# fabianschenk/REVO

Hardware: AMD Instinct MI355X
Metric: tracked frames/sec at 640x480, 4-level pyramid; ATE vs reference (higher is better)
Workload: dtype f32

## Files before the change

revo_amd/csrc/revo_dev.h:

```cpp
#pragma once
#include <hip/hip_runtime.h>
#include <stdint.h>
#include "../../include/revo_hip.h"

#define REVO_L REVO_MAX_LEVELS

struct LevelGeom {
  int w, h;
  int npix;
  float fx, fy, cx, cy;
  int patch;
  int hist_w, hist_h;
  int nchunk;
  int chunk_rows;
  int wpr;
  int nms_block_base;
  int has_orig;
  int pix_base;
  int edt_rows;
  int edt_block_base;
  int strip_base;
  int cc_base;
  int band_rows, nbands, band_base;
};

struct PyrGeom {
  int frame0;
  int n_levels;
  int total_nms_blocks, total_pix, total_edt_blocks, total_strips, total_cc;
  int total_bands, any_banded;
  int hyst_force;
  int hyst_heavy_runs;
  int total_tiles;
  int pts_staged;
  float depth_min, depth_max;
  int canny_low, canny_high;
  int use_edge_hist;
  float n_percentage;
  double fill_thr[REVO_L];
  LevelGeom lv[REVO_L];
};

struct FramePlanes {
  uint8_t* gray[REVO_L];
  float* depth[REVO_L];
  uint2* cs[REVO_L];
  uint8_t* edges[REVO_L];
  uint8_t* edges_orig[REVO_L];
  int* scratch[REVO_L];
  float4* pts[REVO_L];
  float4* pts_trk[REVO_L];
  float* dt[REVO_L];
  float4* table[REVO_L];
  uint8_t* hist[REVO_L];
  int* chunk[REVO_L];
  unsigned* cmask[REVO_L];
  uint8_t* vb[REVO_L];
  int* npts;
  int* hist_nz;
  int* strip_tot;
  uint32_t* ebits[REVO_L];
  int* need_full;
  int* hyst_heavy;
  int* tile_base;
  float* stage[REVO_L];
  unsigned short* epre[REVO_L];
  int* stage_base;
};

struct PairDesc {
  const float4* pts[REVO_L];
  const int* npts;
  const float* dt[REVO_L];
  float R[9];
  float T[3];
};

struct TrackParams {
  int pyr_min_lvl, pyr_max_lvl;
  int lvl_begin, lvl_end;
  int check_init;
  int eval_only;
  int kspec[REVO_L];
  int redundant_n;
  float lambda_success_fac, lambda_fail_fac;
  float lambda_initial[REVO_L], step_size_min[REVO_L], convergence_eps[REVO_L];
  int max_its[REVO_L];
  float edge_distance[REVO_L];
  float huber_edge;
  int use_edge_filter;
  struct { float fx, fy, cx, cy; int w, h; } cam[REVO_L];
  int exact_sums;
};

struct EvalOut {
  float A[36];
  float b[6];
  float error;
  float mean_err;
  float sum_w, sum_u;
  int good, bad;
};

#define REVO_MAX_WIDTH 2048
#define NMS_ROWS 6
#define EDT_ROW_PX 1280
#ifndef REVO_HYST_LDS_MAX
#define REVO_HYST_LDS_MAX 158720
#endif
#ifndef TRACK_THREADS
#define TRACK_THREADS 512
#endif
#ifndef TRACK_MAX_CLUSTER
#define TRACK_MAX_CLUSTER 32
#endif
#define TRACK_KMAX 4
#define TRACK_NVAL 48
#define TRACK_NVAL_X 132
#define TRACK_MAIL_NVAL TRACK_NVAL_X

void launch_gray_depth(const PyrGeom& g, const FramePlanes& p, const uint8_t* d_bgr, const float* d_depth_f32,
                       const uint16_t* d_depth_u16, float u16_alpha, int B, hipStream_t s);
void launch_pyrdown(const PyrGeom& g, const FramePlanes& p, int lvl, int B, hipStream_t s, int parts = 3, bool stage_edges = false);
void launch_edge_prefix(const PyrGeom& g, const FramePlanes& p, int B, hipStream_t s);
void launch_canny_nms(const PyrGeom& g, const FramePlanes& p, int B, hipStream_t s);
void launch_hyst(const PyrGeom& g, const FramePlanes& p, int B, hipStream_t s);
void launch_fill(const PyrGeom& g, const FramePlanes& p, int B, hipStream_t s);
void launch_compact(const PyrGeom& g, const FramePlanes& p, int B, hipStream_t s);
void launch_tile_points(const PyrGeom& g, const FramePlanes& p, int B, hipStream_t s, int which = 3);
void launch_pyrdown_bgr(const uint8_t* src, int w, int h, uint8_t* dst, hipStream_t s);
void launch_colored_pcl(const PyrGeom& g, const FramePlanes& p, int frame, int lvl, int dense, const uint8_t* bgr_lvl,
                        int* chunk, unsigned* cmask, int* total, int cap, float* out8, hipStream_t s);
void launch_keyframe(const PyrGeom& g, const FramePlanes& p, int f0, int fstride, int count, hipStream_t s, int which = 3);
int launch_track(const PairDesc* d_descs, const TrackParams& prm, revo_pair_result* d_out, EvalOut* d_eval,
                 int n_pairs, unsigned long long* d_mail, unsigned* epoch_io, int cluster, unsigned* d_resident, hipStream_t s);
void launch_track_gate(unsigned* d_resident, unsigned want, hipStream_t s);
int launch_track_one(const PairDesc& desc, const TrackParams& prm, revo_pair_result* out, EvalOut* eval_out,
                     unsigned long long* d_mail, unsigned* epoch_io, int cluster, unsigned* seq_ptr, unsigned seq_val,
                     unsigned* d_resident, hipStream_t s);
void launch_solve6(const float* d_Ab , int n, float* d_x , hipStream_t s);
int track_blocks_per_cu();
void launch_grad_table(const PyrGeom& g, const FramePlanes& p, int f0, int fstride, int count, hipStream_t s);
struct VoteArgs { float RT[3][12]; const float4* pts[3]; const int* n[3]; };
void launch_vote(const PyrGeom& g, const FramePlanes& curr, int curr_frame, int lvl, int n_clouds, const VoteArgs& va,
                 int* d_marks , int* d_hist8 , unsigned* d_done ,
                 int* h_out8 , unsigned seq_val, int use_orig_edges,
                 hipStream_t s);
void launch_copy_cloud(float4* dst, const float4* src, int* dst_n, const int* src_n, hipStream_t s);
struct VoteDesc {
  float RT[3][12]; const float4* pts[3]; const int* n[3]; int n_clouds;
  const uint8_t* edges; const float* depth;
  int* marks; int* hist8; unsigned* done;
  int* host_out;
};
struct CloudCopyDesc { float4* dst; const float4* src; int* dst_n; const int* src_n; };
struct CopySeg { const void* src; void* dst; size_t bytes; };
void launch_vote_multi(const PyrGeom& g, int lvl, int n, const VoteDesc* d_descs, unsigned seq_val, hipStream_t s);
void launch_copy_cloud_multi(int n, const CloudCopyDesc* d_descs, hipStream_t s);
void launch_copy_segments(int n, const CopySeg* d_segs, hipStream_t s);
```

revo_amd/csrc/revo_pyramid.hip:

```cpp
#include "revo_dev.h"
#include <type_traits>

namespace {

#ifdef REVO_BUILD_PRIO
#define BUILD_PRIO() __builtin_amdgcn_s_setprio(REVO_BUILD_PRIO)
#else
#define BUILD_PRIO()
#endif

__device__ __forceinline__ int level_of(const PyrGeom& g, int v, int LevelGeom::*base) {
  int l = 0;
#pragma unroll
  for (int k = 1; k < REVO_L; ++k)
    if (k < g.n_levels && v >= g.lv[k].*base) l = k;
  return l;
}
__device__ __forceinline__ int clampi(int v, int lo, int hi) { return v < lo ? lo : (v > hi ? hi : v); }
__device__ __forceinline__ int reflect101(int i, int n) {
  if (i < 0) i = -i;
  if (i >= n) i = 2 * n - 2 - i;
  return i;
}

// ... 74 lines not shown
    if (GRAY && r < 2 * nrows + 3) {
      const uint32_t* row = srcw + (size_t)reflect101(2 * oy - 2 + r, sh) * swords;
      uint32_t w0 = row[max(w1i - 1, 0)];
      const uint32_t w1 = row[w1i], w2 = row[w1i + 1];
      uint32_t w3 = row[min(w1i + 2, swords - 1)];
      if (gx == 0) w0 = (((w1 >> 16) & 0xffu) << 16) | (((w1 >> 8) & 0xffu) << 24);
      if (gx == gw - 1) w3 = (w2 >> 16) & 0xffu;
      const int b[11] = {(int)((w0 >> 16) & 0xffu), (int)(w0 >> 24),
                         (int)(w1 & 0xffu), (int)((w1 >> 8) & 0xffu), (int)((w1 >> 16) & 0xffu), (int)(w1 >> 24),
                         (int)(w2 & 0xffu), (int)((w2 >> 8) & 0xffu), (int)((w2 >> 16) & 0xffu), (int)(w2 >> 24),
                         (int)(w3 & 0xffu)};
#pragma unroll
      for (int j = 0; j < 4; ++j) hs[r][j] = b[2 * j] + b[2 * j + 4] + 4 * (b[2 * j + 1] + b[2 * j + 3]) + 6 * b[2 * j + 2];
    } else {
#pragma unroll
      for (int j = 0; j < 4; ++j) hs[r][j] = 0;
    }
  }
#pragma unroll
  for (int q = 0; q < 2; ++q) {
    if (q >= nrows) break;
    if (GRAY) {
      uint32_t packed = 0;
#pragma unroll
      for (int j = 0; j < 4; ++j) {
        const int v = hs[2 * q][j] + hs[2 * q + 4][j] + 4 * (hs[2 * q + 1][j] + hs[2 * q + 3][j]) + 6 * hs[2 * q + 2][j];
        packed |= (uint32_t)((v + 128) >> 8) << (8 * j);
      }
      reinterpret_cast<uint32_t*>(dst + (size_t)(oy + q) * dw)[gx] = packed;
    }
    if (!DEPTH) continue;
    const float* d0 = dsrc + (size_t)(2 * (oy + q)) * sw + 8 * gx;
    const float4 a0 = *reinterpret_cast<const float4*>(d0), a1 = *reinterpret_cast<const float4*>(d0 + 4);
    const float4 c0 = *reinterpret_cast<const float4*>(d0 + sw), c1 = *reinterpret_cast<const float4*>(d0 + sw + 4);
    const float top[8] = {a0.x, a0.y, a0.z, a0.w, a1.x, a1.y, a1.z, a1.w};
    const float bot[8] = {c0.x, c0.y, c0.z, c0.w, c1.x, c1.y, c1.z, c1.w};
    unsigned vt = 0, vbm = 0;
#pragma unroll
    for (int k = 0; k < 8; ++k) {
      vt |= (isfinite(top[k]) && top[k] > dmin && top[k] < dmax) ? 1u << k : 0u;
      vbm |= (isfinite(bot[k]) && bot[k] > dmin && bot[k] < dmax) ? 1u << k : 0u;
    }
    vsrc[(size_t)(2 * (oy + q)) * (sw >> 3) + gx] = (uint8_t)vt;
    vsrc[(size_t)(2 * (oy + q) + 1) * (sw >> 3) + gx] = (uint8_t)vbm;
    if (STAGE) {
      const int wc = (8 * gx) >> 5, sh8 = (8 * gx) & 31;
#pragma unroll
      for (int rr = 0; rr < 2; ++rr) {
        const int y = 2 * (oy + q) + rr;
        const uint32_t E = es.cs[((size_t)f * sh + y) * es.wpr + wc].y;
        uint32_t eb = (E >> sh8) & 0xffu;
        if (eb) {
          const int tile = (y >> 5) * es.wpr + wc;
          int pos = es.base[(size_t)f * es.tiles_total + tile] + (int)es.epre[((size_t)f * sh + y) * es.wpr + wc] +
                    __popc(E & ((1u << sh8) - 1u));
          float* o = es.out + (size_t)f * sw * sh;
          const float* row = rr ? bot : top;
#pragma unroll
          for (int k = 0; k < 8; ++k)
            if ((eb >> k) & 1u) o[pos++] = row[k];
        }
      }
    }
    float o[4];
#pragma unroll
    for (int j = 0; j < 4; ++j) {
      float out = 0.0f, cnt = 0.0f;
      if (top[2 * j] > 0.0f) { out += top[2 * j]; cnt += 1.0f; }
      if (top[2 * j + 1] > 0.0f) { out += top[2 * j + 1]; cnt += 1.0f; }
      if (bot[2 * j] > 0.0f) { out += bot[2 * j]; cnt += 1.0f; }
      if (bot[2 * j + 1] > 0.0f) { out += bot[2 * j + 1]; cnt += 1.0f; }
      if (cnt > 0.0f) out = __fdiv_rn(out, cnt);
      o[j] = out;
    }
    *reinterpret_cast<float4*>(ddst + (size_t)(oy + q) * dw + 4 * gx) = make_float4(o[0], o[1], o[2], o[3]);
  }
}

typedef short s2v __attribute__((ext_vector_type(2)));
__device__ __forceinline__ s2v as_s2(uint32_t v) { return __builtin_bit_cast(s2v, v); }
__device__ __forceinline__ uint32_t as_u32(s2v v) { return __builtin_bit_cast(uint32_t, v); }
#define PAIR(hi, lo, sel) as_s2(__builtin_amdgcn_perm((hi), (lo), (sel)))

__device__ __forceinline__ void nms_px(int k, int aL, int aM, int aR, int bL, int m, int bR, int cL, int cM, int cR, uint32_t dxy,
                                       int low, int high, uint32_t& cb, uint32_t& sb) {
  const int TG22 = 13573;
  const s2v v = as_s2(dxy);
  const s2v z = {0, 0};
  const uint32_t ab = as_u32(__builtin_elementwise_max(v, z - v));
  const int ax = (int)(ab & 0xffffu);
  const int ay15 = (int)((ab >> 1) & 0x7fff8000u);
  const int t22 = ax * TG22;
  const bool horiz = ay15 < t22;
  const bool vert = ay15 > t22 + (ax << 16);
  const bool neg = (int)(dxy ^ (dxy << 16)) < 0;
  const int diag_a = neg ? aR : aL;
  const int diag_b = neg ? cL : cR;
  const int a = horiz ? bL : (vert ? aM : diag_a);
  const int b = horiz ? bR : (vert ? cM : diag_b);
  const bool ge = horiz || vert;
  const bool is_max = (m > a) & (ge ? (m >= b) : (m > b));
  const bool c = (m > low) & is_max;
  cb |= c ? (1u << k) : 0u;
  sb |= (c & (m > high)) ? (1u << k) : 0u;
}
#define NMS_R 6

struct HRow4 { s2v d[3], s[3]; };
__device__ __forceinline__ HRow4 hrow4(uint32_t prev, uint32_t m0, uint32_t next) {
  const s2v E0 = PAIR(0u, prev, 0x0c030c02u), E1 = PAIR(0u, m0, 0x0c010c00u), E2 = PAIR(0u, m0, 0x0c030c02u), E3 = PAIR(0u, next, 0x0c010c00u);
  const s2v O0 = PAIR(m0, prev, 0x0c040c03u), O1 = PAIR(0u, m0, 0x0c020c01u), O2 = PAIR(next, m0, 0x0c040c03u);
  HRow4 r;
  r.d[0] = E1 - E0; r.d[1] = E2 - E1; r.d[2] = E3 - E2;
  r.s[0] = (E0 + E1) + (O0 + O0); r.s[1] = (E1 + E2) + (O1 + O1); r.s[2] = (E2 + E3) + (O2 + O2);
  return r;
}
struct MRow4 { int v0, v1, v2, v3, v4, v5; };
struct DRow4 { uint32_t v0, v1, v2, v3; };
__device__ __forceinline__ void mag_row4(const HRow4& a, const HRow4& b, const HRow4& c, uint32_t cm_left, uint32_t cm_right, bool valid,
                                         MRow4& m, DRow4& dxy) {
  uint32_t lo[3], hi[3];
#pragma unroll
  for (int k = 0; k < 3; ++k) {
    const s2v dx = (a.d[k] + c.d[k]) + (b.d[k] + b.d[k]);
    const s2v dy = c.s[k] - a.s[k];
    lo[k] = __builtin_amdgcn_perm(as_u32(dy), as_u32(dx), 0x05040100u);
    hi[k] = __builtin_amdgcn_perm(as_u32(dy), as_u32(dx), 0x07060302u);
  }
  const uint32_t rv = valid ? ~0u : 0u;
#define MAG2(x) __builtin_amdgcn_sdot2(as_s2(x), as_s2(x), 0, false)
  m.v0 = MAG2(lo[0]) & (int)(cm_left & rv);
  m.v1 = MAG2(hi[0]) & (int)rv;
  m.v2 = MAG2(lo[1]) & (int)rv;
  m.v3 = MAG2(hi[1]) & (int)rv;
  m.v4 = MAG2(lo[2]) & (int)rv;
  m.v5 = MAG2(hi[2]) & (int)(cm_right & rv);
#undef MAG2
  dxy.v0 = hi[0]; dxy.v1 = lo[1]; dxy.v2 = hi[1]; dxy.v3 = lo[2];
}
__device__ __forceinline__ void nms_row4(const MRow4& A, const MRow4& B, const MRow4& C, const DRow4& d, int low, int high,
                                         uint32_t* cand, uint32_t* strong) {
  uint32_t cb = 0, sb = 0;
  nms_px(0, A.v0, A.v1, A.v2, B.v0, B.v1, B.v2, C.v0, C.v1, C.v2, d.v0, low, high, cb, sb);
  nms_px(1, A.v1, A.v2, A.v3, B.v1, B.v2, B.v3, C.v1, C.v2, C.v3, d.v1, low, high, cb, sb);
  nms_px(2, A.v2, A.v3, A.v4, B.v2, B.v3, B.v4, C.v2, C.v3, C.v4, d.v2, low, high, cb, sb);
  nms_px(3, A.v3, A.v4, A.v5, B.v3, B.v4, B.v5, C.v3, C.v4, C.v5, d.v3, low, high, cb, sb);
  *cand = cb;
  *strong = sb;
}
__global__ void __launch_bounds__(256) k_canny_nms4(PyrGeom g, FramePlanes pl) {
  BUILD_PRIO();
  const int f = g.frame0 + blockIdx.z;
  if (blockIdx.x == 0 && threadIdx.x < REVO_L) {
    pl.need_full[f * REVO_L + threadIdx.x] = 0;
    pl.hist_nz[f * REVO_L + threadIdx.x] = 0;
  }
  const int l = level_of(g, blockIdx.x, &LevelGeom::nms_block_base);
  const LevelGeom& lv = g.lv[l];
  const int w = lv.w, h = lv.h;
  const int rt = 8 * lv.wpr;
  const int t = (blockIdx.x - lv.nms_block_base) * 256 + threadIdx.x;
  const int yb = t / rt, xg = t - yb * rt;
  const int y0 = yb * NMS_R;
  if (y0 >= h) return;
  const int x = xg * 4;
  const bool active = x < w;
  const uint8_t* gray = pl.gray[l] + (size_t)f * lv.npix;
  const bool has_prev = x > 0, has_next = x + 4 < w;
  const int xo = active ? x : 0;
  const int o_prev = (active && has_prev) ? xo - 4 : xo, o_next = (active && has_next) ? xo + 4 : xo;
  const uint32_t cm_left = (active && has_prev) ? ~0u : 0u, cm_right = (active && has_next) ? ~0u : 0u;
  struct Raw { uint32_t prev, m0, next; };
  auto load_raw = [&](int r) -> Raw {
    const int rr = clampi(r, 0, h - 1);
    const uint8_t* row = gray + (size_t)rr * w;
    Raw q;
    q.m0 = *reinterpret_cast<const uint32_t*>(row + xo);
    q.prev = *reinterpret_cast<const uint32_t*>(row + o_prev);
    q.next = *reinterpret_cast<const uint32_t*>(row + o_next);
    return q;
  };
  auto make_hrow = [&](Raw q) -> HRow4 {
    if (!has_prev) q.prev = (q.m0 & 0xffu) * 0x01010101u;
    if (!has_next) q.next = (q.m0 >> 24) * 0x01010101u;
    return hrow4(q.prev, q.m0, q.next);
  };
  HRow4 H0, H1, H2;
  MRow4 M0, M1, M2;
  DRow4 D0, D1, D2;
  {
    const Raw r0 = load_raw(y0 - 2), r1 = load_raw(y0 - 1), r2 = load_raw(y0), r3 = load_raw(y0 + 1);
    H0 = make_hrow(r0); H1 = make_hrow(r1); H2 = make_hrow(r2);
    mag_row4(H0, H1, H2, cm_left, cm_right, active && y0 - 1 >= 0, M0, D0);
    H0 = make_hrow(r3);
  }
  Raw ahead = load_raw(y0 + 2);
  mag_row4(H1, H2, H0, cm_left, cm_right, active, M1, D1);
  uint2* out = pl.cs[l] + ((size_t)f * h + y0) * lv.wpr + (xg >> 3);
  const int sh = 4 * (threadIdx.x & 7);
  auto emit = [&](int i, uint32_t cb, uint32_t sb) {
    uint32_t cw = cb << sh, sw = sb << sh;
    cw |= (uint32_t)__builtin_amdgcn_update_dpp(0, (int)cw, 0xB1, 0xf, 0xf, true);
    sw |= (uint32_t)__builtin_amdgcn_update_dpp(0, (int)sw, 0xB1, 0xf, 0xf, true);
    cw |= (uint32_t)__builtin_amdgcn_update_dpp(0, (int)cw, 0x4E, 0xf, 0xf, true);
    sw |= (uint32_t)__builtin_amdgcn_update_dpp(0, (int)sw, 0x4E, 0xf, 0xf, true);
    cw |= (uint32_t)__builtin_amdgcn_update_dpp(0, (int)cw, 0x141, 0xf, 0xf, true);
    sw |= (uint32_t)__builtin_amdgcn_update_dpp(0, (int)sw, 0x141, 0xf, 0xf, true);
    if ((threadIdx.x & 7) == 0 && y0 + i < h) out[(size_t)i * lv.wpr] = make_uint2(cw, sw);
  };
#define NMS_STEP4(i, Ha, Hb, Hc, Ma, Mb, Mc, Db, Dc)                                  \
  {                                                                                   \
    Hc = make_hrow(ahead);                                                            \
    if ((i) < NMS_R - 1) ahead = load_raw(y0 + (i) + 3);                              \
    mag_row4(Ha, Hb, Hc, cm_left, cm_right, active && y0 + (i) + 1 < h, Mc, Dc);      \
    uint32_t cb, sb;                                                                  \
    nms_row4(Ma, Mb, Mc, Db, g.canny_low, g.canny_high, &cb, &sb);                    \
    emit((i), cb, sb);                                                                \
  }
  NMS_STEP4(0, H2, H0, H1, M0, M1, M2, D1, D2)
  NMS_STEP4(1, H0, H1, H2, M1, M2, M0, D2, D0)
  NMS_STEP4(2, H1, H2, H0, M2, M0, M1, D0, D1)
  NMS_STEP4(3, H2, H0, H1, M0, M1, M2, D1, D2)
  NMS_STEP4(4, H0, H1, H2, M1, M2, M0, D2, D0)
  NMS_STEP4(5, H1, H2, H0, M2, M0, M1, D0, D1)
#undef NMS_STEP4
}

#ifndef HYST_THREADS
#define HYST_THREADS 1024
#endif
__device__ __forceinline__ uint32_t dil3(uint32_t a, uint32_t al, uint32_t ar) {
  return a | __builtin_amdgcn_alignbit(a, al, 31) | __builtin_amdgcn_alignbit(ar, a, 1);
}
__device__ __forceinline__ uint32_t run_fill(uint32_t C, uint32_t S) {
  const uint32_t up = ((C + S) ^ C) & C;
  const uint32_t rC = __builtin_bitreverse32(C), rS = __builtin_bitreverse32(S);
  const uint32_t dn = __builtin_bitreverse32(((rC + rS) ^ rC) & rC);
  return up | dn | S;
}

#ifdef REVO_HYST_PROFILE
#define HP(i) if (threadIdx.x == 0) hp[i] = clock64()
#define HA(i) if (threadIdx.x == 0) { const long long now_ = clock64(); ha[i] += now_ - hlast; hlast = now_; }
#else
#define HP(i)
#define HA(i)
#endif
template <bool C_IN_LDS, bool E_GLOBAL = false>
__device__ __forceinline__ void hyst_level(const PyrGeom& g, const FramePlanes& pl, const int l, const int f, uint32_t* s_mem) {
  static_assert(!(C_IN_LDS && E_GLOBAL), "the candidate bitmap is in LDS only when the edge bitmap is");
#ifdef REVO_HYST_PROFILE
  long long hp[12], ha[8], hlast = 0;
  for (int i = 0; i < 12; ++i) hp[i] = 0;
  for (int i = 0; i < 8; ++i) ha[i] = 0;
  int dbg_sweeps = 0, dbg_bands = 0;
#endif
  HP(0);
  const LevelGeom& lv = g.lv[l];
  const int w = lv.w, h = lv.h, wpr = lv.wpr;
  const int pitch = wpr;
  const int nwords = h * wpr;
  const int e_words = (h + 2) * pitch + 2;
  uint32_t* Cl = s_mem;
  uint32_t* Ebase = C_IN_LDS ? s_mem + (REVO_HYST_LDS_MAX / 4 - e_words)
                  : (E_GLOBAL ? reinterpret_cast<uint32_t*>(pl.scratch[l] + (size_t)f * g.lv[l].npix) : s_mem);
  uint32_t* E = Ebase + 1;
  const uint2* cs = pl.cs[l] + (size_t)f * h * wpr;
  const int tid = threadIdx.x;
  for (int i = tid; i < pitch + 1; i += HYST_THREADS) { Ebase[i] = 0u; Ebase[e_words - 1 - i] = 0u; }
  for (int i = tid; i < nwords; i += HYST_THREADS) {
    const uint2 v = cs[i];
    E[pitch + i] = v.y;
    if (C_IN_LDS) Cl[i] = v.x & ~v.y;
  }
  __syncthreads();
  HP(1);
  bool done = false;
#ifdef REVO_HYST_PROFILE
  int dbg_runs = -1, dbg_t = 0, dbg_a = 0;
#endif
  if (C_IN_LDS) {
    unsigned short* Bs = reinterpret_cast<unsigned short*>(Cl + nwords);
    uint32_t* parent = Cl + nwords + (nwords + 2) / 2;
    const int table_words = (int)(REVO_HYST_LDS_MAX / 4) - (nwords + (nwords + 2) / 2);
    const int cap = min(table_words / 2, table_words - e_words);
    const int cap_keep = (table_words - e_words) / 2;
    __shared__ int s_wsum[HYST_THREADS / 64];
    __shared__ int s_total, s_promoted;
#ifdef REVO_HYST_PROFILE
    __shared__ int s_dbg[4];
    if (tid < 4) s_dbg[tid] = 0;
#endif
    auto weak = [&](int wi) -> uint32_t { return Cl[wi]; };
    auto starts = [](uint32_t wk) -> uint32_t { return wk & ~(wk << 1); };
    const float inv_wpr = 1.0f / (float)wpr;
    const uint32_t FLAG = 0x80000000u, IDM = 0x7fffffffu;
#ifdef REVO_HYST_PROFILE
    hlast = clock64();
#endif
    for (int sweep = 0; sweep < 64 && !done; ++sweep) {
#ifdef REVO_HYST_PROFILE
      ++dbg_sweeps;
#endif
      {
        const int wpt = (nwords + HYST_THREADS - 1) / HYST_THREADS;
        const int w0 = min(nwords, tid * wpt), w1 = min(nwords, w0 + wpt);
        int mine = 0;
// ... 1299 lines not shown
  }
}

__global__ void __launch_bounds__(1024) k_pcl_scan(int* chunk, int n, int* total) {
  __shared__ int s_part[1024];
  const int t = block_exclusive_scan(chunk, n, s_part);
  if (threadIdx.x == 0) *total = t;
}

#define EDT_INF (1 << 29)
#define EDT_THREADS 1024
#define EDT_COL_GROUPS(h) ((h) > 1024 ? 64 : ((h) > 512 ? 32 : 16))
__global__ void __launch_bounds__(EDT_THREADS) k_edt_cols(PyrGeom g, FramePlanes pl, int f0, int fstride, int nframes) {
  __shared__ int s_first[EDT_THREADS];
  __shared__ int s_last[EDT_THREADS];
  const int f = f0 + (blockIdx.x % nframes) * fstride;
  int l = 0, sidx = blockIdx.x / nframes, ngroups = 16, ncols = 64;
  for (int k = 0; k < g.n_levels; ++k) {
    ngroups = EDT_COL_GROUPS(g.lv[k].h);
    ncols = EDT_THREADS / ngroups;
    const int ns = (g.lv[k].w + ncols - 1) / ncols;
    if (sidx < ns) { l = k; break; }
    sidx -= ns;
  }
  const LevelGeom& lv = g.lv[l];
  const int col = threadIdx.x % ncols, grp = threadIdx.x / ncols;
  const int x = sidx * ncols + col;
  const int rpg = (lv.h + ngroups - 1) / ngroups;
  const int yb = min(lv.h, grp * rpg), ye = min(lv.h, yb + rpg);
  const bool in = x < lv.w;
  const uint8_t* edges = pl.edges[l] + (size_t)f * lv.npix;
  unsigned em = 0;
  if ((lv.w & 31) == 0 && (ncols & 31) == 0) {
    const uint2* csw = pl.cs[l] + (size_t)f * lv.h * lv.wpr;
    const int r = threadIdx.x & 31;
    const int wc = (sidx * ncols + (col & ~31)) >> 5;
    uint32_t v = 0;
    if (yb + r < ye && wc < lv.wpr) v = csw[(size_t)(yb + r) * lv.wpr + wc].y;
    em = tile_transpose32(v, r);
    if (!in) em = 0;
  } else if (in) {
#pragma unroll 8
    for (int y = yb; y < ye; ++y) em |= (edges[(size_t)y * lv.w + x] ? 1u : 0u) << (y - yb);
  }
  s_first[grp * ncols + col] = em ? yb + __ffs(em) - 1 : EDT_INF;
  s_last[grp * ncols + col] = em ? yb + 31 - __clz(em) : -EDT_INF;
  __syncthreads();
  if (!in) return;
  int above = -EDT_INF, below = EDT_INF;
  for (int k = 0; k < grp; ++k) above = max(above, s_last[k * ncols + col]);
  for (int k = ngroups - 1; k > grp; --k) below = min(below, s_first[k * ncols + col]);
  uint16_t* gd = reinterpret_cast<uint16_t*>(pl.scratch[l]) + (size_t)f * lv.npix;
  const int FAR = 1 << 20;
  int du = (above <= -EDT_INF) ? FAR : (yb - above);
  const int dbelow = (below >= EDT_INF) ? FAR : (below - yb);
  for (int y = yb; y < ye; ++y) {
    const int k = y - yb;
    const unsigned hi = em >> k;
    du = (hi & 1u) ? 0 : du;
    const int dn = hi ? __ffs(hi) - 1 : dbelow - k;
    const int m = min(du, dn);
    gd[(size_t)y * lv.w + x] = (uint16_t)(m >= 0xffff ? 0xffff : m);
    du += 1;
  }
}

__device__ __forceinline__ float sqrt_rn_int(float x) {
  const float s = __builtin_amdgcn_sqrtf(x);
  const unsigned si = __float_as_uint(s);
  const float sd = __uint_as_float(si - 1u), su = __uint_as_float(si + 1u);
  const float rd = __builtin_fmaf(-sd, s, x), ru = __builtin_fmaf(-su, s, x);
  float r = (rd <= 0.0f) ? sd : s;
  r = (ru > 0.0f) ? su : r;
  return r;
}
__global__ void __launch_bounds__(256) k_edt_rows(PyrGeom g, FramePlanes pl, int f0, int fstride) {
  extern __shared__ int s_g2[];
  const int f = f0 + blockIdx.z * fstride;
  const int l = level_of(g, blockIdx.x, &LevelGeom::edt_block_base);
  const LevelGeom lv = g.lv[l];
  const int w = lv.w;
  const int y0 = (blockIdx.x - lv.edt_block_base) * lv.edt_rows;
  const int nr = min(lv.edt_rows, lv.h - y0);
  const int pad = w + 4, pitch = w + 2 * pad;
  const uint16_t* gd = reinterpret_cast<const uint16_t*>(pl.scratch[l]) + (size_t)f * lv.npix + (size_t)y0 * w;
  const int4 inf4 = make_int4(EDT_INF, EDT_INF, EDT_INF, EDT_INF);
  const int padq = pad >> 2, wq = w >> 2;
  for (int r = 0; r < nr; ++r) {
    int4* row4 = reinterpret_cast<int4*>(s_g2 + r * pitch);
    for (int i = threadIdx.x; i < padq; i += 256) { row4[i] = inf4; row4[padq + wq + i] = inf4; }
    const uint2* src = reinterpret_cast<const uint2*>(gd + r * w);
    for (int i = threadIdx.x; i < wq; i += 256) {
      const uint2 q = src[i];
      const int d0 = (int)(q.x & 0xffffu), d1 = (int)(q.x >> 16), d2 = (int)(q.y & 0xffffu), d3 = (int)(q.y >> 16);
      row4[padq + i] = make_int4(d0 == 0xffff ? EDT_INF : __mul24(d0, d0), d1 == 0xffff ? EDT_INF : __mul24(d1, d1),
                                 d2 == 0xffff ? EDT_INF : __mul24(d2, d2), d3 == 0xffff ? EDT_INF : __mul24(d3, d3));
    }
  }
  __syncthreads();
  float* dt = pl.dt[l] + (size_t)f * lv.npix + (size_t)y0 * w;
  const int dq = 256 / w, dr = 256 - dq * w;
  int r = threadIdx.x / w, x = threadIdx.x - r * w;
  for (int p = threadIdx.x; p < nr * w; p += 256) {
    const int* c = s_g2 + r * pitch + pad + x;
    int best = c[0];
    for (int d = 1; d < w && d * d < best; d += 4) {
      int m = best;
#pragma unroll
      for (int j = 0; j < 4; ++j) {
        const int dj = d + j;
        m = min(m, dj * dj + min(c[-dj], c[dj]));
      }
      best = m;
    }
    dt[p] = best >= EDT_INF ? sqrtf(1e15f) : sqrt_rn_int((float)best);
    x += dr; r += dq;
    if (x >= w) { x -= w; ++r; }
  }
}

__global__ void __launch_bounds__(256) k_grad_table(PyrGeom g, FramePlanes pl, int f0, int fstride) {
  const int f = f0 + blockIdx.z * fstride;
  const int l = blockIdx.y;
  const LevelGeom& lv = g.lv[l];
  const int i = blockIdx.x * 256 + threadIdx.x;
  if (i >= lv.npix) return;
  const float* dt = pl.dt[l] + (size_t)f * lv.npix;
  float4 o = make_float4(0.f, 0.f, 0.f, 0.f);
  if (i >= lv.w && i < lv.w * (lv.h - 1)) {
    o.x = 0.5f * (dt[i - 1] - dt[i + 1]);
    o.y = 0.5f * (dt[i - lv.w] - dt[i + lv.w]);
    o.z = dt[i];
  }
  pl.table[l][(size_t)f * lv.npix + i] = o;
}

__global__ void __launch_bounds__(256) k_vote_mark(VoteArgs a, float fx, float fy, float cx, float cy, int W, int H,
                                                   int* marks) {
  const int c = blockIdx.y;
  const int n = *a.n[c];
  const float* R = a.RT[c];
  const float* T = R + 9;
  const float4* pts = a.pts[c];
  for (int i = blockIdx.x * 256 + threadIdx.x; i < n; i += gridDim.x * 256) {
    const float4 p = pts[i];
    float q[3];
#pragma unroll
    for (int r = 0; r < 3; ++r) q[r] = ((R[r] * p.x + R[3 + r] * p.y) + R[6 + r] * p.z) + T[r];
    const float u = __fdiv_rn(fx * q[0], q[2]) + cx;
    const float v = __fdiv_rn(fy * q[1], q[2]) + cy;
    if (u >= 0 && u < (float)W && v >= 0 && v < (float)H)
      atomicOr(&marks[(int)floorf(v) * W + (int)floorf(u)], 1 << c);
  }
}

__global__ void __launch_bounds__(256) k_vote_hist(int* marks, const uint8_t* edges, const float* depth, int npix,
                                                   float dmin, float dmax, int* hist8, unsigned* done, int* host_out,
                                                   unsigned seq_val) {
  __shared__ int s_h[8];
  __shared__ bool s_last;
  if (threadIdx.x < 8) s_h[threadIdx.x] = 0;
  __syncthreads();
  for (int i = blockIdx.x * 256 + threadIdx.x; i < npix; i += gridDim.x * 256) {
    const int m = marks[i];
    if (m) marks[i] = 0;
    const float Z = depth[i];
    if (depth_ok(Z, dmin, dmax)) {
      const int val = __popc(m);
      atomicAdd(&s_h[val], 1);
      if (edges[i] > 0) atomicAdd(&s_h[4 + val], 1);
    }
  }
  __syncthreads();
  if (threadIdx.x < 8 && s_h[threadIdx.x]) atomicAdd(&hist8[threadIdx.x], s_h[threadIdx.x]);
  __threadfence();
  __syncthreads();
  if (threadIdx.x == 0) s_last = (atomicAdd(done, 1u) == gridDim.x - 1);
  __syncthreads();
  if (s_last) {
    if (threadIdx.x < 8) host_out[threadIdx.x] = atomicExch(&hist8[threadIdx.x], 0);
    if (threadIdx.x == 0) *done = 0u;
    __threadfence_system();
    __syncthreads();
    if (threadIdx.x == 0) *(volatile int*)&host_out[8] = (int)seq_val;
  }
}

__global__ void __launch_bounds__(256) k_copy_cloud(float4* __restrict__ dst, const float4* __restrict__ src,
                                                    int* __restrict__ dst_n, const int* __restrict__ src_n) {
  const int n = *src_n;
  for (int i = blockIdx.x * 256 + threadIdx.x; i < n; i += gridDim.x * 256) dst[i] = src[i];
  if (blockIdx.x == 0 && threadIdx.x == 0) *dst_n = n;
}

// ... 152 lines not shown
  }
  const bool mixed = !banded && fits_single && g.hyst_heavy_runs > 0 && g.total_bands > 0 && g.lv[0].nbands > 1;
  if (mixed) {
    static bool attr3 = false;
    if (!attr3) {
      (void)hipFuncSetAttribute(reinterpret_cast<const void*>(k_hyst_mixed), hipFuncAttributeMaxDynamicSharedMemorySize, REVO_HYST_LDS_MAX);
      (void)hipFuncSetAttribute(reinterpret_cast<const void*>(k_hyst_out), hipFuncAttributeMaxDynamicSharedMemorySize, HB_LDS_WORDS * 4);
      (void)hipFuncSetAttribute(reinterpret_cast<const void*>(k_hyst_seam), hipFuncAttributeMaxDynamicSharedMemorySize, 64 * 1024);
      (void)hipGetLastError();
      attr3 = true;
    }
    const LevelGeom& l0 = g.lv[0];
    const size_t seam_lds = std::max<size_t>(4, (size_t)l0.nbands * (size_t)(HB_LDS_WORDS / 2 / 32 + 64) * 4);
    const size_t out_lds = std::max<size_t>(4, (size_t)l0.band_rows * l0.wpr * 4);
    hipLaunchKernelGGL(k_hyst_mixed, dim3((l0.nbands + g.n_levels) * B), dim3(HYST_THREADS), REVO_HYST_LDS_MAX, s, g, p, B);
    hipLaunchKernelGGL(k_hyst_seam, dim3(B), dim3(HS_THREADS), seam_lds, s, g, p, 1);
    hipLaunchKernelGGL(k_hyst_out, dim3(l0.nbands * B), dim3(HO_THREADS), out_lds, s, g, p, 1);
    hipLaunchKernelGGL(k_hyst<true>, dim3(std::min(32, g.n_levels * B)), dim3(HYST_THREADS), REVO_HYST_LDS_MAX, s, g, p, 1, B);
    return;
  }
  const int n_wg = only_flagged ? std::min(32, g.n_levels * B) : g.n_levels * B;
  if (ec_bytes + 4096 <= REVO_HYST_LDS_MAX)
    hipLaunchKernelGGL(k_hyst<true>, dim3(n_wg), dim3(HYST_THREADS), REVO_HYST_LDS_MAX, s, g, p, only_flagged, B);
  else if (e_bytes <= REVO_HYST_LDS_MAX)
    hipLaunchKernelGGL(k_hyst<false>, dim3(n_wg), dim3(HYST_THREADS), e_bytes, s, g, p, only_flagged, B);
  else
    hipLaunchKernelGGL((k_hyst<false, true>), dim3(n_wg), dim3(HYST_THREADS), 16, s, g, p, only_flagged, B);
}

void launch_fill(const PyrGeom& g, const FramePlanes& p, int B, hipStream_t s) {
  bool any = false;
  for (int l = 1; l < g.n_levels; ++l) any = any || g.lv[l].has_orig;
  if (!any) return;
  if (g.lv[0].npix <= 640 * 480) {
    hipLaunchKernelGGL(k_fill, dim3(1, 1, B), dim3(1024), 0, s, g, p, 0);
    return;
  }
  for (int l = 1; l < g.n_levels; ++l) {
    if (!g.lv[l].has_orig) continue;
    const int n = (g.lv[l - 1].w / 2) * (g.lv[l - 1].h / 2);
    hipLaunchKernelGGL(k_fill, dim3(std::min(64, (n + 1023) / 1024), 1, B), dim3(1024), 0, s, g, p, l);
  }
}

void launch_tile_points(const PyrGeom& g, const FramePlanes& p, int B, hipStream_t s, int which) {
  if (which & 1) hipLaunchKernelGGL(k_tile_count, dim3(g.n_levels * B), dim3(1024), 0, s, g, p);
  const int groups = (g.total_tiles + PT_TILES - 1) / PT_TILES;
  if ((which & 2) && g.pts_staged) hipLaunchKernelGGL(k_pts_tiles<true>, dim3(groups * B), dim3(32 * PT_TILES), 0, s, g, p);
  else if (which & 2) hipLaunchKernelGGL(k_pts_tiles<false>, dim3(groups * B), dim3(32 * PT_TILES), 0, s, g, p);
}

void launch_compact(const PyrGeom& g, const FramePlanes& p, int B, hipStream_t s) {
  dim3 grid(g.total_strips * B);
  hipLaunchKernelGGL(k_compact_walk<false>, grid, dim3(CW_COLS * CW_LANES_COUNT), 0, s, g, p);
  hipLaunchKernelGGL(k_compact_walk<true>, grid, dim3(CW_COLS * CW_LANES), 0, s, g, p);
}

void launch_pyrdown_bgr(const uint8_t* src, int w, int h, uint8_t* dst, hipStream_t s) {
  hipLaunchKernelGGL(k_pyrdown_bgr, dim3(((w / 2) * (h / 2) + 255) / 256), dim3(256), 0, s, src, w, h, dst);
}

void launch_colored_pcl(const PyrGeom& g, const FramePlanes& p, int frame, int lvl, int dense, const uint8_t* bgr_lvl,
                        int* chunk, unsigned* cmask, int* total, int cap, float* out8, hipStream_t s) {
  const LevelGeom& lv = g.lv[lvl];
  const float* depth = p.depth[lvl] + (size_t)frame * lv.npix;
  const uint8_t* edges = p.edges[lvl] + (size_t)frame * lv.npix;
  const int n = lv.w * lv.nchunk;
  dim3 grid((n + 255) / 256);
  hipLaunchKernelGGL(k_pcl_walk<false>, grid, dim3(256), 0, s, lv, g.depth_min, g.depth_max, depth, edges, bgr_lvl, dense,
                     chunk, cmask, total, cap, (float4*)out8);
  hipLaunchKernelGGL(k_pcl_scan, dim3(1), dim3(1024), 0, s, chunk, n, total);
  hipLaunchKernelGGL(k_pcl_walk<true>, grid, dim3(256), 0, s, lv, g.depth_min, g.depth_max, depth, edges, bgr_lvl, dense,
                     chunk, cmask, total, cap, (float4*)out8);
}

void launch_keyframe(const PyrGeom& g, const FramePlanes& p, int f0, int fstride, int count, hipStream_t s, int which) {
  int strips = 0;
  for (int l = 0; l < g.n_levels; ++l) {
    const int ncols = EDT_THREADS / EDT_COL_GROUPS(g.lv[l].h);
    strips += (g.lv[l].w + ncols - 1) / ncols;
  }
  if (which & 1) hipLaunchKernelGGL(k_edt_cols, dim3(strips * count), dim3(EDT_THREADS), 0, s, g, p, f0, fstride, count);
  size_t rows_lds = 0;
  for (int l = 0; l < g.n_levels; ++l) rows_lds = std::max(rows_lds, (size_t)g.lv[l].edt_rows * (3 * g.lv[l].w + 8) * sizeof(int));
  if (which & 2) hipLaunchKernelGGL(k_edt_rows, dim3(g.total_edt_blocks, 1, count), dim3(256), rows_lds, s, g, p, f0, fstride);
}

void launch_grad_table(const PyrGeom& g, const FramePlanes& p, int f0, int fstride, int count, hipStream_t s) {
  hipLaunchKernelGGL(k_grad_table, dim3((g.lv[0].npix + 255) / 256, g.n_levels, count), dim3(256), 0, s, g, p, f0, fstride);
}

void launch_vote(const PyrGeom& g, const FramePlanes& curr, int curr_frame, int lvl, int n_clouds, const VoteArgs& va,
                 int* d_marks, int* d_hist8, unsigned* d_done, int* h_out8, unsigned seq_val, int use_orig_edges, hipStream_t s) {
  const LevelGeom& lv = g.lv[lvl];
  if (n_clouds > 0)
    hipLaunchKernelGGL(k_vote_mark, dim3(32, n_clouds), dim3(256), 0, s, va, lv.fx, lv.fy, lv.cx, lv.cy, lv.w, lv.h, d_marks);
  const uint8_t* edges = (use_orig_edges ? curr.edges_orig[lvl] : curr.edges[lvl]) + (size_t)curr_frame * lv.npix;
  hipLaunchKernelGGL(k_vote_hist, dim3(16), dim3(256), 0, s, d_marks, edges,
                     curr.depth[lvl] + (size_t)curr_frame * lv.npix, lv.npix, g.depth_min, g.depth_max, d_hist8, d_done, h_out8,
                     seq_val);
}

void launch_copy_cloud(float4* dst, const float4* src, int* dst_n, const int* src_n, hipStream_t s) {
  hipLaunchKernelGGL(k_copy_cloud, dim3(16), dim3(256), 0, s, dst, src, dst_n, src_n);
}

void launch_vote_multi(const PyrGeom& g, int lvl, int n, const VoteDesc* d_descs, unsigned seq_val, hipStream_t s) {
  const LevelGeom& lv = g.lv[lvl];
  hipLaunchKernelGGL(k_vote_mark_multi, dim3(32, 3, n), dim3(256), 0, s, d_descs, lv.fx, lv.fy, lv.cx, lv.cy, lv.w, lv.h);
  hipLaunchKernelGGL(k_vote_hist_multi, dim3(16, n), dim3(256), 0, s, d_descs, lv.npix, g.depth_min, g.depth_max, seq_val);
}

void launch_copy_cloud_multi(int n, const CloudCopyDesc* d_descs, hipStream_t s) {
  hipLaunchKernelGGL(k_copy_cloud_multi, dim3(16, n), dim3(256), 0, s, d_descs);
}

void launch_copy_segments(int n, const CopySeg* d_segs, hipStream_t s) {
  hipLaunchKernelGGL(k_copy_segments, dim3(64, n), dim3(256), 0, s, d_segs);
}
```

Baseline: 109,700.

## Double Canny NMS rows per thread, branch-free borders, wider EDT row search

Doubles the rows each Canny NMS thread processes and rolls the step macros into an unrolled loop. It also replaces the border handling with perm-selectors and sdot2 accumulator masks, and simplifies the direction tests and bit packing. Separately, the EDT row pass now scans 8 offsets per iteration with incremental squares and a wave-wide __any exit, which needs wider LDS padding. These cut per-pixel ALU work and per-thread overhead, but risk fewer blocks for parallelism at small pyramid levels and more wasted work from the wave-uniform early exit.

```diff
diff --git a/revo_amd/csrc/revo_dev.h b/revo_amd/csrc/revo_dev.h
--- a/revo_amd/csrc/revo_dev.h
+++ b/revo_amd/csrc/revo_dev.h
@@ -103,7 +103,7 @@
 };
 
 #define REVO_MAX_WIDTH 2048
-#define NMS_ROWS 6
+#define NMS_ROWS 12
 #define EDT_ROW_PX 1280
 #ifndef REVO_HYST_LDS_MAX
 #define REVO_HYST_LDS_MAX 158720
diff --git a/revo_amd/csrc/revo_pyramid.hip b/revo_amd/csrc/revo_pyramid.hip
--- a/revo_amd/csrc/revo_pyramid.hip
+++ b/revo_amd/csrc/revo_pyramid.hip
@@ -180,34 +180,35 @@
 __device__ __forceinline__ uint32_t as_u32(s2v v) { return __builtin_bit_cast(uint32_t, v); }
 #define PAIR(hi, lo, sel) as_s2(__builtin_amdgcn_perm((hi), (lo), (sel)))
 
-__device__ __forceinline__ void nms_px(int k, int aL, int aM, int aR, int bL, int m, int bR, int cL, int cM, int cR, uint32_t dxy,
+__device__ __forceinline__ void nms_px(int aL, int aM, int aR, int bL, int m, int bR, int cL, int cM, int cR, uint32_t dxy,
                                        int low, int high, uint32_t& cb, uint32_t& sb) {
   const int TG22 = 13573;
   const s2v v = as_s2(dxy);
   const s2v z = {0, 0};
   const uint32_t ab = as_u32(__builtin_elementwise_max(v, z - v));
   const int ax = (int)(ab & 0xffffu);
-  const int ay15 = (int)((ab >> 1) & 0x7fff8000u);
-  const int t22 = ax * TG22;
-  const bool horiz = ay15 < t22;
-  const bool vert = ay15 > t22 + (ax << 16);
+  const int ay16 = (int)(ab & 0xffff0000u);
+  const bool horiz = ay16 < ax * (2 * TG22);
+  const bool vert = ay16 > ax * (2 * TG22 + (2 << 16));
   const bool neg = (int)(dxy ^ (dxy << 16)) < 0;
   const int diag_a = neg ? aR : aL;
   const int diag_b = neg ? cL : cR;
   const int a = horiz ? bL : (vert ? aM : diag_a);
   const int b = horiz ? bR : (vert ? cM : diag_b);
-  const bool ge = horiz || vert;
-  const bool is_max = (m > a) & (ge ? (m >= b) : (m > b));
+  const int mb = (horiz || vert) ? m + 1 : m;
+  const bool is_max = (m > a) & (mb > b);
   const bool c = (m > low) & is_max;
-  cb |= c ? (1u << k) : 0u;
-  sb |= (c & (m > high)) ? (1u << k) : 0u;
-}
-#define NMS_R 6
+  cb = cb + cb + (c ? 1u : 0u);
+  sb = sb + sb + ((c & (m > high)) ? 1u : 0u);
+}
+#define NMS_R NMS_ROWS
+static_assert(NMS_R % 3 == 0, "k_canny_nms4 rotates its row registers in threes");
 
 struct HRow4 { s2v d[3], s[3]; };
-__device__ __forceinline__ HRow4 hrow4(uint32_t prev, uint32_t m0, uint32_t next) {
-  const s2v E0 = PAIR(0u, prev, 0x0c030c02u), E1 = PAIR(0u, m0, 0x0c010c00u), E2 = PAIR(0u, m0, 0x0c030c02u), E3 = PAIR(0u, next, 0x0c010c00u);
-  const s2v O0 = PAIR(m0, prev, 0x0c040c03u), O1 = PAIR(0u, m0, 0x0c020c01u), O2 = PAIR(next, m0, 0x0c040c03u);
+struct HSel { uint32_t e0, o0, e3, o2; };
+__device__ __forceinline__ HRow4 hrow4(uint32_t prev, uint32_t m0, uint32_t next, const HSel& q) {
+  const s2v E0 = PAIR(prev, m0, q.e0), E1 = PAIR(0u, m0, 0x0c010c00u), E2 = PAIR(0u, m0, 0x0c030c02u), E3 = PAIR(next, m0, q.e3);
+  const s2v O0 = PAIR(prev, m0, q.o0), O1 = PAIR(0u, m0, 0x0c020c01u), O2 = PAIR(next, m0, q.o2);
   HRow4 r;
   r.d[0] = E1 - E0; r.d[1] = E2 - E1; r.d[2] = E3 - E2;
   r.s[0] = (E0 + E1) + (O0 + O0); r.s[1] = (E1 + E2) + (O1 + O1); r.s[2] = (E2 + E3) + (O2 + O2);
@@ -215,7 +216,8 @@
 }
 struct MRow4 { int v0, v1, v2, v3, v4, v5; };
 struct DRow4 { uint32_t v0, v1, v2, v3; };
-__device__ __forceinline__ void mag_row4(const HRow4& a, const HRow4& b, const HRow4& c, uint32_t cm_left, uint32_t cm_right, bool valid,
+#define NMS_OUT (-(1 << 30))
+__device__ __forceinline__ void mag_row4(const HRow4& a, const HRow4& b, const HRow4& c, int acc_l, int acc_r, int acc_m,
                                          MRow4& m, DRow4& dxy) {
   uint32_t lo[3], hi[3];
 #pragma unroll
@@ -225,24 +227,23 @@
     lo[k] = __builtin_amdgcn_perm(as_u32(dy), as_u32(dx), 0x05040100u);
     hi[k] = __builtin_amdgcn_perm(as_u32(dy), as_u32(dx), 0x07060302u);
   }
-  const uint32_t rv = valid ? ~0u : 0u;
-#define MAG2(x) __builtin_amdgcn_sdot2(as_s2(x), as_s2(x), 0, false)
-  m.v0 = MAG2(lo[0]) & (int)(cm_left & rv);
-  m.v1 = MAG2(hi[0]) & (int)rv;
-  m.v2 = MAG2(lo[1]) & (int)rv;
-  m.v3 = MAG2(hi[1]) & (int)rv;
-  m.v4 = MAG2(lo[2]) & (int)rv;
-  m.v5 = MAG2(hi[2]) & (int)(cm_right & rv);
+#define MAG2(x, acc) __builtin_amdgcn_sdot2(as_s2(x), as_s2(x), (acc), false)
+  m.v0 = MAG2(lo[0], acc_l | acc_m);
+  m.v1 = MAG2(hi[0], acc_m);
+  m.v2 = MAG2(lo[1], acc_m);
+  m.v3 = MAG2(hi[1], acc_m);
+  m.v4 = MAG2(lo[2], acc_m);
+  m.v5 = MAG2(hi[2], acc_r | acc_m);
 #undef MAG2
   dxy.v0 = hi[0]; dxy.v1 = lo[1]; dxy.v2 = hi[1]; dxy.v3 = lo[2];
 }
 __device__ __forceinline__ void nms_row4(const MRow4& A, const MRow4& B, const MRow4& C, const DRow4& d, int low, int high,
                                          uint32_t* cand, uint32_t* strong) {
   uint32_t cb = 0, sb = 0;
-  nms_px(0, A.v0, A.v1, A.v2, B.v0, B.v1, B.v2, C.v0, C.v1, C.v2, d.v0, low, high, cb, sb);
-  nms_px(1, A.v1, A.v2, A.v3, B.v1, B.v2, B.v3, C.v1, C.v2, C.v3, d.v1, low, high, cb, sb);
-  nms_px(2, A.v2, A.v3, A.v4, B.v2, B.v3, B.v4, C.v2, C.v3, C.v4, d.v2, low, high, cb, sb);
-  nms_px(3, A.v3, A.v4, A.v5, B.v3, B.v4, B.v5, C.v3, C.v4, C.v5, d.v3, low, high, cb, sb);
+  nms_px(A.v3, A.v4, A.v5, B.v3, B.v4, B.v5, C.v3, C.v4, C.v5, d.v3, low, high, cb, sb);
+  nms_px(A.v2, A.v3, A.v4, B.v2, B.v3, B.v4, C.v2, C.v3, C.v4, d.v2, low, high, cb, sb);
+  nms_px(A.v1, A.v2, A.v3, B.v1, B.v2, B.v3, C.v1, C.v2, C.v3, d.v1, low, high, cb, sb);
+  nms_px(A.v0, A.v1, A.v2, B.v0, B.v1, B.v2, C.v0, C.v1, C.v2, d.v0, low, high, cb, sb);
   *cand = cb;
   *strong = sb;
 }
@@ -267,7 +268,8 @@
   const bool has_prev = x > 0, has_next = x + 4 < w;
   const int xo = active ? x : 0;
   const int o_prev = (active && has_prev) ? xo - 4 : xo, o_next = (active && has_next) ? xo + 4 : xo;
-  const uint32_t cm_left = (active && has_prev) ? ~0u : 0u, cm_right = (active && has_next) ? ~0u : 0u;
+  const int acc_l = has_prev ? 0 : NMS_OUT, acc_r = has_next ? 0 : NMS_OUT, acc_lane = active ? 0 : NMS_OUT;
+  const int low = max(g.canny_low, 0);
   struct Raw { uint32_t prev, m0, next; };
   auto load_raw = [&](int r) -> Raw {
     const int rr = clampi(r, 0, h - 1);
@@ -278,22 +280,23 @@
     q.next = *reinterpret_cast<const uint32_t*>(row + o_next);
     return q;
   };
-  auto make_hrow = [&](Raw q) -> HRow4 {
-    if (!has_prev) q.prev = (q.m0 & 0xffu) * 0x01010101u;
-    if (!has_next) q.next = (q.m0 >> 24) * 0x01010101u;
-    return hrow4(q.prev, q.m0, q.next);
-  };
+  HSel sel;
+  sel.e0 = has_prev ? 0x0c070c06u : 0x0c000c00u;
+  sel.o0 = has_prev ? 0x0c000c07u : 0x0c000c00u;
+  sel.e3 = has_next ? 0x0c050c04u : 0x0c030c03u;
+  sel.o2 = has_next ? 0x0c040c03u : 0x0c030c03u;
+  auto make_hrow = [&](Raw q) -> HRow4 { return hrow4(q.prev, q.m0, q.next, sel); };
   HRow4 H0, H1, H2;
   MRow4 M0, M1, M2;
   DRow4 D0, D1, D2;
   {
     const Raw r0 = load_raw(y0 - 2), r1 = load_raw(y0 - 1), r2 = load_raw(y0), r3 = load_raw(y0 + 1);
     H0 = make_hrow(r0); H1 = make_hrow(r1); H2 = make_hrow(r2);
-    mag_row4(H0, H1, H2, cm_left, cm_right, active && y0 - 1 >= 0, M0, D0);
+    mag_row4(H0, H1, H2, acc_l, acc_r, y0 - 1 >= 0 ? acc_lane : NMS_OUT, M0, D0);
     H0 = make_hrow(r3);
   }
   Raw ahead = load_raw(y0 + 2);
-  mag_row4(H1, H2, H0, cm_left, cm_right, active, M1, D1);
+  mag_row4(H1, H2, H0, acc_l, acc_r, acc_lane, M1, D1);
   uint2* out = pl.cs[l] + ((size_t)f * h + y0) * lv.wpr + (xg >> 3);
   const int sh = 4 * (threadIdx.x & 7);
   auto emit = [&](int i, uint32_t cb, uint32_t sb) {
@@ -310,17 +313,17 @@
   {                                                                                   \
     Hc = make_hrow(ahead);                                                            \
     if ((i) < NMS_R - 1) ahead = load_raw(y0 + (i) + 3);                              \
-    mag_row4(Ha, Hb, Hc, cm_left, cm_right, active && y0 + (i) + 1 < h, Mc, Dc);      \
+    mag_row4(Ha, Hb, Hc, acc_l, acc_r, y0 + (i) + 1 < h ? acc_lane : NMS_OUT, Mc, Dc); \
     uint32_t cb, sb;                                                                  \
-    nms_row4(Ma, Mb, Mc, Db, g.canny_low, g.canny_high, &cb, &sb);                    \
+    nms_row4(Ma, Mb, Mc, Db, low, g.canny_high, &cb, &sb);                            \
     emit((i), cb, sb);                                                                \
   }
-  NMS_STEP4(0, H2, H0, H1, M0, M1, M2, D1, D2)
-  NMS_STEP4(1, H0, H1, H2, M1, M2, M0, D2, D0)
-  NMS_STEP4(2, H1, H2, H0, M2, M0, M1, D0, D1)
-  NMS_STEP4(3, H2, H0, H1, M0, M1, M2, D1, D2)
-  NMS_STEP4(4, H0, H1, H2, M1, M2, M0, D2, D0)
-  NMS_STEP4(5, H1, H2, H0, M2, M0, M1, D0, D1)
+#pragma unroll
+  for (int i = 0; i < NMS_R; i += 3) {
+    NMS_STEP4(i, H2, H0, H1, M0, M1, M2, D1, D2)
+    NMS_STEP4(i + 1, H0, H1, H2, M1, M2, M0, D2, D0)
+    NMS_STEP4(i + 2, H1, H2, H0, M2, M0, M1, D0, D1)
+  }
 #undef NMS_STEP4
 }
 
@@ -1786,7 +1789,7 @@
   const int w = lv.w;
   const int y0 = (blockIdx.x - lv.edt_block_base) * lv.edt_rows;
   const int nr = min(lv.edt_rows, lv.h - y0);
-  const int pad = w + 4, pitch = w + 2 * pad;
+  const int pad = w + 8, pitch = w + 2 * pad;
   const uint16_t* gd = reinterpret_cast<const uint16_t*>(pl.scratch[l]) + (size_t)f * lv.npix + (size_t)y0 * w;
   const int4 inf4 = make_int4(EDT_INF, EDT_INF, EDT_INF, EDT_INF);
   const int padq = pad >> 2, wq = w >> 2;
@@ -1808,12 +1811,13 @@
   for (int p = threadIdx.x; p < nr * w; p += 256) {
     const int* c = s_g2 + r * pitch + pad + x;
     int best = c[0];
-    for (int d = 1; d < w && d * d < best; d += 4) {
+    for (int d = 1, dd = 1; d < w && __any(dd < best); dd += 16 * d + 64, d += 8) {
       int m = best;
-#pragma unroll
-      for (int j = 0; j < 4; ++j) {
-        const int dj = d + j;
-        m = min(m, dj * dj + min(c[-dj], c[dj]));
+      int sq = dd, dsq = 2 * d + 1;
+#pragma unroll
+      for (int j = 0; j < 8; ++j) {
+        m = min(m, sq + min(c[-(d + j)], c[d + j]));
+        sq += dsq; dsq += 2;
       }
       best = m;
     }
@@ -2132,7 +2136,7 @@
   }
   if (which & 1) hipLaunchKernelGGL(k_edt_cols, dim3(strips * count), dim3(EDT_THREADS), 0, s, g, p, f0, fstride, count);
   size_t rows_lds = 0;
-  for (int l = 0; l < g.n_levels; ++l) rows_lds = std::max(rows_lds, (size_t)g.lv[l].edt_rows * (3 * g.lv[l].w + 8) * sizeof(int));
+  for (int l = 0; l < g.n_levels; ++l) rows_lds = std::max(rows_lds, (size_t)g.lv[l].edt_rows * (3 * g.lv[l].w + 16) * sizeof(int));
   if (which & 2) hipLaunchKernelGGL(k_edt_rows, dim3(g.total_edt_blocks, 1, count), dim3(256), rows_lds, s, g, p, f0, fstride);
 }
 
```

Result: no change. 109,800 (median of 3 runs) (+0.1%).
